# TobiaMarcucci/warm-start-hybrid-mpc

Measured on NVIDIA B200. Metric: bnb_qp_relaxations_per_s, higher is better.
Workload: dtype f64

## Files before the change

warm-start-hybrid-mpc_b200/csrc/qp_device.cuh:

```cuda
#pragma once
#include <cuda_runtime.h>
#include <math.h>
#include <stdint.h>

#ifndef WS_TU
#define WS_TU_HAS(id) 1
#else
#define WS_TU_HAS(id) (WS_TU == (id))
#endif

#ifndef WS_NT
#define WS_NT 256
#endif
#ifndef WS_MAXL
#define WS_MAXL 2
#endif
#define WS_NW (WS_NT / 32)
#ifndef WS_RPT
#define WS_RPT ((384 + WS_NT - 1) / WS_NT)
#endif
#ifndef WS_RRT
#define WS_RRT (256 / WS_NT)
#endif
#ifndef WS_NOINLINE
#define WS_NOINLINE __forceinline__
#endif
#if defined(WS_TU) && WS_TU % 2 == 1
#define WS_WIDE_REGS 1
#else
#define WS_WIDE_REGS 0
#endif
#ifndef WS_CH
#if WS_WIDE_REGS
#define WS_CH 4
#else
#define WS_CH 2
#endif
#endif
#if !WS_WIDE_REGS && !defined(WS_PRICE8)
#define WS_PRICE4 1
#endif
#define WS_OPTIMAL 2
#define WS_INFEASIBLE 3
#define WS_ITER_LIMIT 9
#define WS_REORTH 1e-2
#define WS_LAM_MAX 1e13

#define WS_TID ((int)(threadIdx.x & (WS_NT - 1)))
#define WS_LANE ((int)(threadIdx.x / WS_NT))
#define WS_SYNC() asm volatile("bar.sync %0, %1;" :: "r"(WS_LANE + 1), "n"(WS_NT) : "memory")

struct SmemOff {
    int z, c1, c2, t, u, ls, lam, cw, yc, wv, v, bu, blb, xi, part, red;
    int vf0, vf;
    int pool, pool_sz;
    int irow, iside, ired, iscr;
    int idep;
    int ints;
    int binW, bign, bnadd;
    int bytes;
    int lane_doubles;
    int t_inr, t_vsc, t_sF, t_sG, t_sF1, t_sG1, t_rinfo;
    int tab_doubles;
    int total_bytes;
};

struct DevProblem {
    int nx, nu, nub, nuc, T, nh, nh1, nq, nqT, nr, n, m, mc, nb, ns;
    const double *A, *B, *F, *G, *h, *F1, *G1, *h1, *Q, *R, *QT, *Mmu, *MmuT, *Mrho;
    const double *Mh, *WfT, *nrm, *inr, *vscale, *Eh, *hh, *Rinv, *RinvT, *Kx, *ZmapT, *Linv, *LinvT, *Msq;
    const int *bin_idx;
    int n_elim;
    int search_rule;
    const int *border;
    double eps, tol_p, tol_d, tol_sing, tol_ray, prox_tol;
    int max_iter, max_prox;
    int lanes;
    int ld;
    int np;
    int ns2;
    int gp;
    int hot_cap;
    SmemOff so;
    int n_primal, n_dual, off_lam, off_mu, off_nulb, off_nuub, off_rho, off_sigma;
    int n_rec;
    int node_rule;
};

#ifdef WS_PROF
__device__ unsigned long long g_prof[256];
__device__ __forceinline__ void prof_mark(int id) {
    __shared__ long long s_prof_last;
    if (threadIdx.x == 0) {
        const long long t = clock64();
        atomicAdd(&g_prof[2 * id], (unsigned long long)(t - s_prof_last)); atomicAdd(&g_prof[2 * id + 1], 1ull);
        s_prof_last = clock64();
    }
}
__device__ __forceinline__ void prof_add(int id, int value) {
    if (threadIdx.x == 0) { atomicAdd(&g_prof[2 * id], (unsigned long long)value); atomicAdd(&g_prof[2 * id + 1], 1ull); }
}
#else
#define prof_mark(id) ((void)0)
#define prof_add(id, value) ((void)0)
#endif

__host__ __device__ __forceinline__ int tri_off(int j) { return j * (j + 1) / 2; }

struct SlotPtrs {
    double *Q;
    double *Ri;
    double *lam;
    double *yc;
    int *row;
    int *side;
    int *nW;
};

__host__ __device__ __forceinline__ size_t slot_doubles(int n, int ld) { return (((size_t)n * ld + (size_t)tri_off(n) + (n + 1) + n + 4) + 1) & ~(size_t)1; }
__host__ __device__ __forceinline__ size_t slot_ints(int n) { return 2 * (size_t)(n + 1) + 4; }

__device__ __forceinline__ SlotPtrs slot_ptrs(double *dbase, int *ibase, int slot, int n, int ld) {
    SlotPtrs s;
    double *d = dbase + (size_t)slot * slot_doubles(n, ld);
    int *i = ibase + (size_t)slot * slot_ints(n);
    s.Q = d; d += (size_t)n * ld;
    s.Ri = d; d += tri_off(n);
    s.lam = d; d += n + 1;
    s.yc = d;
    s.row = i; i += n + 1;
    s.side = i; i += n + 1;
    s.nW = i;
    return s;
}

struct Ctx {
    double *smd;
    double *tab;
    double *gQ, *gRi;
    int pg, prp;
};

#define SMV(name) (cx.smd + P.so.name)
#define SMI(name) (reinterpret_cast<int *>(cx.smd + P.so.ints) + P.so.name)
#define SMB(name) (reinterpret_cast<unsigned char *>(cx.smd + P.so.bytes) + P.so.name)
#define TBV(name) (cx.tab + P.so.t_##name)
#define TBI(name) (reinterpret_cast<const int *>(cx.tab + P.so.t_##name))

__device__ __forceinline__ Ctx make_ctx(const DevProblem &P, unsigned char *smem_raw, const SlotPtrs &sp) {
    Ctx cx;
    cx.tab = reinterpret_cast<double *>(smem_raw);
    cx.smd = cx.tab + P.so.tab_doubles + (size_t)WS_LANE * P.so.lane_doubles;
    cx.gQ = sp.Q; cx.gRi = sp.Ri;
    const int hs = P.ns2 >> 1;
    cx.pg = WS_TID / hs; cx.prp = WS_TID - cx.pg * hs;
    return cx;
}

struct Geom {
    int d;
    int d0;
    int he;
    int ldc;
    int ks;
    int triR;
    int G, W;
};

__device__ __forceinline__ Geom load_geom(const DevProblem &P, const Ctx &cx) {
    const int *g = SMI(idep);
    Geom q;
    q.d = g[0]; q.d0 = g[2]; q.he = g[3]; q.ldc = g[4]; q.ks = g[5]; q.triR = g[6]; q.G = g[7]; q.W = g[8];
    return q;
}

__device__ __forceinline__ void store_geom(const DevProblem &P, const Ctx &cx, int d) {
    int *g = SMI(idep);
    d = d < P.n_elim ? d : P.n_elim;
    const int d0 = d & ~1, he = (P.np - d0) >> 1, ldc = 2 * (he | 1);
    int ks = P.n - d;
    while (ks > 0 && (size_t)ks * ldc + ((tri_off(ks) + 1) & ~1) > (size_t)P.so.pool_sz) --ks;
    const int G = he <= WS_NT ? (WS_NT / he < 8 ? WS_NT / he : 8) : 1;
    g[0] = d; g[2] = d0; g[3] = he; g[4] = ldc; g[5] = ks; g[6] = (tri_off(ks) + 1) & ~1; g[7] = G; g[8] = WS_NT / G;
}

__device__ __forceinline__ double warp_sum(double x) {
#pragma unroll
    for (int o = 16; o > 0; o >>= 1) x += __shfl_xor_sync(0xffffffffu, x, o);
    return x;
}

#define WS_FULL 0xffffffffu
static_assert(WS_NW == 16 || WS_NW == 8 || WS_NW == 4 || WS_NW == 2, "the two-level reductions assume 2, 4, 8 or 16 warps per CTA");

__device__ __forceinline__ double block_sum(double x, double *red) {
    const int lane = WS_TID & 31, w = WS_TID >> 5;
    x = warp_sum(x);
    WS_SYNC();
    if (lane == 0) red[w] = x;
    WS_SYNC();
    double s = lane < WS_NW ? red[lane] : 0.;
#pragma unroll
    for (int o = WS_NW / 2; o > 0; o >>= 1) s += __shfl_xor_sync(WS_FULL, s, o);
    return __shfl_sync(WS_FULL, s, 0);
}

__device__ __forceinline__ void block_sum2(double &x, double &y, double *red) {
    const int lane = WS_TID & 31, w = WS_TID >> 5;
    x = warp_sum(x); y = warp_sum(y);
    WS_SYNC();
    if (lane == 0) { red[w] = x; red[16 + w] = y; }
    WS_SYNC();
    double s = (lane & 15) < WS_NW ? red[lane] : 0.;
#pragma unroll
    for (int o = 8; o > 0; o >>= 1) s += __shfl_xor_sync(WS_FULL, s, o);
    x = __shfl_sync(WS_FULL, s, 0); y = __shfl_sync(WS_FULL, s, 16);
}

__device__ __forceinline__ bool better_max(double ov, int oi, double val, int idx) {
    return oi >= 0 && (idx < 0 || ov > val || (ov == val && oi < idx));
}

__device__ __forceinline__ void block_argmax(double &val, int &idx, double *red, int *ired) {
    const int lane = WS_TID & 31, w = WS_TID >> 5;
#pragma unroll
    for (int o = 16; o > 0; o >>= 1) {
        const double ov = __shfl_xor_sync(WS_FULL, val, o);
        const int oi = __shfl_xor_sync(WS_FULL, idx, o);
        if (better_max(ov, oi, val, idx)) { val = ov; idx = oi; }
    }
    WS_SYNC();
    if (lane == 0) { red[w] = val; ired[w] = idx; }
    WS_SYNC();
    val = lane < WS_NW ? red[lane] : 0.; idx = lane < WS_NW ? ired[lane] : -1;
#pragma unroll
    for (int o = WS_NW / 2; o > 0; o >>= 1) {
        const double ov = __shfl_xor_sync(WS_FULL, val, o);
        const int oi = __shfl_xor_sync(WS_FULL, idx, o);
        if (better_max(ov, oi, val, idx)) { val = ov; idx = oi; }
    }
    val = __shfl_sync(WS_FULL, val, 0); idx = __shfl_sync(WS_FULL, idx, 0);
}

__device__ __forceinline__ double block_max(double x, double *red) {
    const int lane = WS_TID & 31, w = WS_TID >> 5;
#pragma unroll
    for (int o = 16; o > 0; o >>= 1) x = fmax(x, __shfl_xor_sync(WS_FULL, x, o));
    WS_SYNC();
    if (lane == 0) red[w] = x;
    WS_SYNC();
    double s = lane < WS_NW ? red[lane] : 0.;
#pragma unroll
    for (int o = WS_NW / 2; o > 0; o >>= 1) s = fmax(s, __shfl_xor_sync(WS_FULL, s, o));
    return __shfl_sync(WS_FULL, s, 0);
}

__device__ __forceinline__ void block_argmin(double &val, int &idx, double *red, int *ired) {
    double nv = -val;
    block_argmax(nv, idx, red, ired);
    val = -nv;
}

__device__ __forceinline__ void warp_argmin_sum(double &val, int &idx, double &sum) {
    double nv = -val;
#pragma unroll
    for (int o = 16; o > 0; o >>= 1) {
        const double ov = __shfl_xor_sync(WS_FULL, nv, o);
        const int oi = __shfl_xor_sync(WS_FULL, idx, o);
        sum += __shfl_xor_sync(WS_FULL, sum, o);
        if (better_max(ov, oi, nv, idx)) { nv = ov; idx = oi; }
    }
    val = -nv;
}

__device__ __forceinline__ void block_argmin_sum(double &val, int &idx, double &sum, double *red, int *ired) {
    const int lane = WS_TID & 31, w = WS_TID >> 5;
    double nv = -val;
#pragma unroll
    for (int o = 16; o > 0; o >>= 1) {
        const double ov = __shfl_xor_sync(WS_FULL, nv, o);
        const int oi = __shfl_xor_sync(WS_FULL, idx, o);
        sum += __shfl_xor_sync(WS_FULL, sum, o);
        if (better_max(ov, oi, nv, idx)) { nv = ov; idx = oi; }
    }
    WS_SYNC();
    if (lane == 0) { red[w] = nv; ired[w] = idx; red[16 + w] = sum; }
    WS_SYNC();
    nv = lane < WS_NW ? red[lane] : 0.; idx = lane < WS_NW ? ired[lane] : -1;
    sum = lane < WS_NW ? red[16 + lane] : 0.;
#pragma unroll
    for (int o = WS_NW / 2; o > 0; o >>= 1) {
        const double ov = __shfl_xor_sync(WS_FULL, nv, o);
        const int oi = __shfl_xor_sync(WS_FULL, idx, o);
        sum += __shfl_xor_sync(WS_FULL, sum, o);
        if (better_max(ov, oi, nv, idx)) { nv = ov; idx = oi; }
    }
    val = -__shfl_sync(WS_FULL, nv, 0); idx = __shfl_sync(WS_FULL, idx, 0); sum = __shfl_sync(WS_FULL, sum, 0);
}

template <class Out>
__device__ __forceinline__ void grouped_matvec(const double *__restrict__ M, int ld, int rows, int j0, int j1,
                                      const double *x, double *part, Out out) {
    if (rows <= WS_NT) {
        const int G = WS_NT / rows;
        const int g = WS_TID / rows, i = WS_TID - g * rows;
        if (g < G) {
            double s0 = 0., s1 = 0., s2 = 0., s3 = 0.;
            int j = j0 + g;
            for (; j + 7 * G < j1; j += 8 * G) {
                double w[8];
#pragma unroll
                for (int q = 0; q < 8; ++q) w[q] = __ldg(M + (size_t)(j + q * G) * ld + i);
                s0 += w[0] * x[j] + w[4] * x[j + 4 * G];
                s1 += w[1] * x[j + G] + w[5] * x[j + 5 * G];
                s2 += w[2] * x[j + 2 * G] + w[6] * x[j + 6 * G];
                s3 += w[3] * x[j + 3 * G] + w[7] * x[j + 7 * G];
            }
            for (; j + 3 * G < j1; j += 4 * G) {
                s0 += M[(size_t)j * ld + i] * x[j];
                s1 += M[(size_t)(j + G) * ld + i] * x[j + G];
                s2 += M[(size_t)(j + 2 * G) * ld + i] * x[j + 2 * G];
                s3 += M[(size_t)(j + 3 * G) * ld + i] * x[j + 3 * G];
            }
            for (; j < j1; j += G) s0 += M[(size_t)j * ld + i] * x[j];
            part[g * rows + i] = (s0 + s1) + (s2 + s3);
        }
        WS_SYNC();
        if (WS_TID < rows) {
            double s = part[WS_TID];
            for (int q = 1; q < G; ++q) s += part[q * rows + WS_TID];
            out(WS_TID, s);
        }
        WS_SYNC();
    } else {
        for (int i = WS_TID; i < rows; i += WS_NT) {
            double s0 = 0., s1 = 0., s2 = 0., s3 = 0.;
            int j = j0;
            for (; j + 7 < j1; j += 8) {
                double w[8];
#pragma unroll
                for (int q = 0; q < 8; ++q) w[q] = __ldg(M + (size_t)(j + q) * ld + i);
                s0 += w[0] * x[j] + w[4] * x[j + 4];
                s1 += w[1] * x[j + 1] + w[5] * x[j + 5];
                s2 += w[2] * x[j + 2] + w[6] * x[j + 6];
                s3 += w[3] * x[j + 3] + w[7] * x[j + 7];
            }
            for (; j < j1; ++j) s0 += M[(size_t)j * ld + i] * x[j];
            out(i, (s0 + s1) + (s2 + s3));
        }
        WS_SYNC();
    }
}

__device__ __forceinline__ double *pool_Ri(const DevProblem &P, const Ctx &cx) { return SMV(pool); }
template <bool SM>
__device__ __forceinline__ double *qcol_w(const DevProblem &P, const Ctx &cx, const Geom &g, int j) {
    if (SM) return SMV(pool) + g.triR + j * g.ldc - g.d0;
    return (j < g.ks ? SMV(pool) + g.triR + j * g.ldc : cx.gQ + (size_t)j * P.ld) - g.d0;
}
template <bool SM>
__device__ __forceinline__ double *ricol_w(const DevProblem &P, const Ctx &cx, const Geom &g, int j) {
    if (SM) return SMV(pool) + tri_off(j);
    return (j < g.ks ? SMV(pool) : cx.gRi) + tri_off(j);
}

__device__ __forceinline__ int team_log2(int k) { return k >= WS_NT ? 0 : min(5, 31 - __clz(WS_NT / max(k, 1))); }

__device__ __forceinline__ double team_sum(double s, int lg) {
    for (int o = 32 >> lg; o < 32; o <<= 1) s += __shfl_xor_sync(0xffffffffu, s, o);
    return s;
}

template <bool SM>
__device__ __forceinline__ void qt_dots_t(const DevProblem &P, const Ctx &cx, int k, const double *x, double *out) {
    const Geom gm = load_geom(P, cx);
    const int lg = team_log2(k), ng = 1 << lg, C = 32 >> lg, jw = WS_NT >> lg;
    const int lane = WS_TID & 31, g = lane >> (5 - lg), jl = (WS_TID >> 5) * C + (lane & (C - 1));
    const int p0 = (gm.d0 >> 1) + g, p1 = P.np >> 1;
    const double2 *x2 = reinterpret_cast<const double2 *>(x);
    const int kr = (k + jw - 1) / jw * jw;
    for (int j = jl; j < kr; j += jw) {
        double s0 = 0., s1 = 0.;
        if (j < k) {
            const double2 *q2 = reinterpret_cast<const double2 *>(qcol_w<SM>(P, cx, gm, j));
            for (int p = p0; p < p1; p += ng) { const double2 a = q2[p], b = x2[p]; s0 += a.x * b.x; s1 += a.y * b.y; }
        }
        const double s = team_sum(s0 + s1, lg);
        if (g == 0 && j < k) out[j] = s;
    }
    WS_SYNC();
}

template <bool SM>
__device__ __forceinline__ double q_apply_t(const DevProblem &P, const Ctx &cx, int k, const double *c, const double *zin, double *zout,
                                 double extra = 0., double *extra_sum = nullptr) {
    const Geom gm = load_geom(P, cx);
    double2 *part2 = reinterpret_cast<double2 *>(SMV(part));
    const int G = gm.G, W = gm.W, he = gm.he, dh = gm.d0 >> 1;
    const int grp = WS_TID / W, t = WS_TID - grp * W;
    if (grp < G) {
        for (int pp = t; pp < he; pp += W) {
            double ax = 0., ay = 0., bx = 0., by = 0.;
            int j = grp;
            for (; j + G < k; j += 2 * G) {
                const double2 a = reinterpret_cast<const double2 *>(qcol_w<SM>(P, cx, gm, j))[dh + pp];
                const double2 b = reinterpret_cast<const double2 *>(qcol_w<SM>(P, cx, gm, j + G))[dh + pp];
                const double ca = c[j], cb = c[j + G];
                ax += a.x * ca; ay += a.y * ca; bx += b.x * cb; by += b.y * cb;
            }
            if (j < k) { const double2 a = reinterpret_cast<const double2 *>(qcol_w<SM>(P, cx, gm, j))[dh + pp]; const double ca = c[j]; ax += a.x * ca; ay += a.y * ca; }
            part2[grp * he + pp] = make_double2(ax + bx, ay + by);
        }
    }
    WS_SYNC();
    const double *part = SMV(part);
    double zz = 0.;
    for (int i = WS_TID; i < 2 * he; i += WS_NT) {
        double s = part[i];
        for (int q = 1; q < G; ++q) s += part[q * 2 * he + i];
        const double zi = (zin ? zin[gm.d0 + i] : 0.) - s;
        zout[gm.d0 + i] = zi; zz += zi * zi;
    }
    {
        const int lane = WS_TID & 31, w = WS_TID >> 5;
        double *red = SMV(red) + 72;
        zz = warp_sum(zz); extra = warp_sum(extra);
        if (lane == 0) { red[w] = zz; red[16 + w] = extra; }
        WS_SYNC();
        double sv = (lane & 15) < WS_NW ? red[lane] : 0.;
#pragma unroll
        for (int o = 8; o > 0; o >>= 1) sv += __shfl_xor_sync(WS_FULL, sv, o);
        zz = __shfl_sync(WS_FULL, sv, 0);
        if (extra_sum) *extra_sum = __shfl_sync(WS_FULL, sv, 16);
    }
    return zz;
}

template <bool SM, class Out>
__device__ __forceinline__ void ri_matvec_ep(const DevProblem &P, const Ctx &cx, int k, const double *c, Out out) {
    const Geom gm = load_geom(P, cx);
    const int lg = team_log2(k), ng = 1 << lg, C = 32 >> lg, jw = WS_NT >> lg;
    const int lane = WS_TID & 31, g = lane >> (5 - lg), il = (WS_TID >> 5) * C + (lane & (C - 1));
    const int kr = (k + jw - 1) / jw * jw;
    for (int i = il; i < kr; i += jw) {
        double s0 = 0., s1 = 0.;
        if (i < k) {
            int j = i + g;
            for (; j + ng < k; j += 2 * ng) { s0 += ricol_w<SM>(P, cx, gm, j)[i] * c[j]; s1 += ricol_w<SM>(P, cx, gm, j + ng)[i] * c[j + ng]; }
            if (j < k) s0 += ricol_w<SM>(P, cx, gm, j)[i] * c[j];
        }
        const double sv = team_sum(s0 + s1, lg);
        if (g == 0 && i < k) out(i, sv);
    }
}

template <bool SM>
__device__ __forceinline__ void ri_matvec(const DevProblem &P, const Ctx &cx, int k, const double *c, double *t) {
    ri_matvec_ep<SM>(P, cx, k, c, [&](int i, double s) { t[i] = s; });
    WS_SYNC();
}

template <bool SM>
__device__ __forceinline__ void rit_matvec_t(const DevProblem &P, const Ctx &cx, int k, const double *d, double *u) {
    const Geom gm = load_geom(P, cx);
    const int lg = team_log2(k), ng = 1 << lg, C = 32 >> lg, jw = WS_NT >> lg;
    const int lane = WS_TID & 31, g = lane >> (5 - lg), jl = (WS_TID >> 5) * C + (lane & (C - 1));
    const int kr = (k + jw - 1) / jw * jw;
    for (int j = jl; j < kr; j += jw) {
        double s = 0.;
        if (j < k) { const double *col = ricol_w<SM>(P, cx, gm, j); for (int i = g; i <= j; i += ng) s += col[i] * d[i]; }
        s = team_sum(s, lg);
        if (g == 0 && j < k) u[j] = s;
    }
    WS_SYNC();
}

__device__ __forceinline__ double neg_bound(const DevProblem &P, const Ctx &cx, int r, int s) {
    return -(s > 0 ? SMV(bu)[r] : -SMV(blb)[r - P.mc]);
}

__device__ __forceinline__ void refresh_uv(const DevProblem &P, const Ctx &cx, int k) {
    const Geom gm = load_geom(P, cx);
    const int *row = SMI(irow), *side = SMI(iside);
    for (int i = WS_TID; i < k; i += WS_NT) SMV(cw)[i] = neg_bound(P, cx, row[i], side[i]);
    for (int i = WS_TID; i < P.np; i += WS_NT) SMV(v)[i] = 0.;
    WS_SYNC();
    if (k <= gm.ks) { rit_matvec_t<true>(P, cx, k, SMV(cw), SMV(u)); ri_matvec<true>(P, cx, k, SMV(u), SMV(ls)); q_apply_t<true>(P, cx, k, SMV(u), nullptr, SMV(v)); }
    else { rit_matvec_t<false>(P, cx, k, SMV(cw), SMV(u)); ri_matvec<false>(P, cx, k, SMV(u), SMV(ls)); q_apply_t<false>(P, cx, k, SMV(u), nullptr, SMV(v)); }
}

struct RowEnt { double e[WS_RPT]; };

__device__ __forceinline__ RowEnt load_row_entries(const DevProblem &P, int r, int d, int d0) {
    RowEnt x;
#pragma unroll
    for (int q = 0; q < WS_RPT; ++q) {
        const int i = d0 + WS_TID + q * WS_NT;
        x.e[q] = (i < P.n && i >= d) ? __ldg(P.Mh + (size_t)r * P.n + i) : 0.;
    }
    return x;
}

template <bool SM>
__device__ __forceinline__ int thin_append_t(const DevProblem &P, const Ctx &cx, int &k, int r, int sgn, bool track, const RowEnt *pre = nullptr) {
    const Geom gm = load_geom(P, cx);
    const int n = P.n, d = gm.d;
    if (k >= WS_RRT * WS_NT) return -1;
    double *z = SMV(z), *c1 = SMV(c1), *t = SMV(t);
    const int pb = track ? 30 : 40;
    (void)pb;
    {
        const RowEnt e = pre ? *pre : load_row_entries(P, r, d, gm.d0);
#pragma unroll
        for (int q = 0; q < WS_RPT; ++q) { const int i = gm.d0 + WS_TID + q * WS_NT; if (i < P.np) z[i] = (double)sgn * e.e[q]; }
    }
    WS_SYNC();
    prof_mark(pb);
    qt_dots_t<SM>(P, cx, k, z, c1);
    prof_mark(pb + 1);
    double cu = 0.;
    if (track) for (int j = WS_TID; j < k; j += WS_NT) cu += c1[j] * SMV(u)[j];
    double rho2 = q_apply_t<SM>(P, cx, k, c1, z, z, cu, &cu);
    prof_mark(pb + 2);
    if (k > 0 && rho2 < WS_REORTH * __ldg(P.Msq + (size_t)r * (P.nb + 1) + d)) {
        double *c2 = SMV(c2);
        qt_dots_t<SM>(P, cx, k, z, c2);
        double cu2 = 0.;
        for (int j = WS_TID; j < k; j += WS_NT) { const double dc = c2[j]; c1[j] += dc; if (track) cu2 += dc * SMV(u)[j]; }
        rho2 = q_apply_t<SM>(P, cx, k, c2, z, z, cu2, &cu2);
        cu += cu2;
        prof_mark(pb + 4);
    }
    const bool dep = k >= n - d || rho2 <= P.tol_sing * P.tol_sing;
    const double ir = dep ? 0. : 1. / sqrt(rho2);
    double *qk = qcol_w<SM>(P, cx, gm, k), *rk = ricol_w<SM>(P, cx, gm, k);
    double uk = 0., lk = 0.;
    if (track && !dep) { uk = (neg_bound(P, cx, r, sgn) - cu) * ir; lk = uk * ir; }
    ri_matvec_ep<SM>(P, cx, k, c1, [&](int i, double ti) {
        t[i] = ti;
        if (!dep) { rk[i] = -ti * ir; if (track) SMV(ls)[i] -= ti * lk; }
    });
    if (dep) { WS_SYNC(); prof_mark(pb + 5); return 0; }
    for (int i = gm.d0 + WS_TID; i < P.np; i += WS_NT) {
        const double q = z[i] * ir;
        qk[i] = q;
        if (track) SMV(v)[i] -= q * uk;
    }
    if (WS_TID == 0) {
        rk[k] = ir;
        SMI(irow)[k] = r; SMI(iside)[k] = sgn; SMV(lam)[k] = 0.;
        if (track) { SMV(u)[k] = uk; SMV(ls)[k] = lk; }
    }
    k += 1;
    if (track) WS_SYNC();
    prof_mark(pb + 6);
    return 1;
}

template <bool SM>
__device__ __forceinline__ int thin_remove_t(const DevProblem &P, const Ctx &cx, int &k, int kp) {
    const Geom gm = load_geom(P, cx);
    auto QC = [&](int j) -> double * { return qcol_w<SM>(P, cx, gm, j); };
    auto RC = [&](int j) -> double * { return ricol_w<SM>(P, cx, gm, j); };
    const int lane = WS_TID & 31, w = WS_TID >> 5, tid = WS_TID;
    double *gc = SMV(c2), *gs = SMV(cw), *u = SMV(u);
    int *row = SMI(irow), *side = SMI(iside), *flag = SMI(ired) + 32;
    if (tid == 0) *flag = 0x7fffffff;
    prof_add(100, k - 1 - kp);
    prof_add(101, k);
    if (kp == k - 1) {
        const double ul = u[kp];
        const double *qk = QC(kp);
        for (int i = gm.d0 + tid; i < P.np; i += WS_NT) SMV(v)[i] += qk[i] * ul;
        const double *rl = RC(kp);
        for (int i = tid; i < kp; i += WS_NT) SMV(ls)[i] -= rl[i] * ul;
        k -= 1;
        WS_SYNC();
        prof_mark(50);
        return -1;
    }
    if (w == 0) {
        const double wkp = RC(kp)[kp];
        double run = 0.;
        for (int b = kp; b < k; b += 32) {
            const int j = b + lane;
            const double wj = j < k ? RC(j)[kp] : 0.;
            double s = wj * wj;
#pragma unroll
            for (int o = 1; o < 32; o <<= 1) { const double y = __shfl_up_sync(0xffffffffu, s, o); if (lane >= o) s += y; }
            s += run;
            double excl = __shfl_up_sync(0xffffffffu, s, 1);
            if (lane == 0) excl = run;
            if (j > kp && j < k) {
                const double isj = 1. / sqrt(s);
                const double tau = (j - 1 == kp) ? wkp : sqrt(excl);
                gc[j - 1] = wj * isj; gs[j - 1] = -tau * isj;
            }
            run = __shfl_sync(0xffffffffu, s, 31);
        }
    }
    int rw[WS_RRT], sd[WS_RRT]; double lm[WS_RRT];
#pragma unroll
    for (int q = 0; q < WS_RRT; ++q) {
        const int ts = kp + 1 + tid + q * WS_NT;
        rw[q] = 0; sd[q] = 0; lm[q] = 0.;
        if (ts < k) { rw[q] = row[ts]; sd[q] = side[ts]; lm[q] = SMV(lam)[ts]; }
    }
    int qr[WS_RPT]; double qcarry[WS_RPT];
#pragma unroll
    for (int q = 0; q < WS_RPT; ++q) { const int i = gm.d0 + tid + q * WS_NT; qr[q] = i < P.np ? i : -1; }
    int rr[WS_RRT], ro[WS_RRT]; double rcarry[WS_RRT], ls_old[WS_RRT];
#pragma unroll
    for (int q = 0; q < WS_RRT; ++q) {
        const int r = WS_NT - 1 - tid + q * WS_NT;
        rr[q] = r < k - 1 ? r : -1;
        ro[q] = r < kp ? r : r + 1;
    }
    const int nq1 = (2 * gm.he + 31) & ~31;
    const bool uth = tid == (nq1 < WS_NT ? nq1 : 0);
    const double big = 1. / P.tol_sing;
    WS_SYNC();
    prof_mark(51);
#pragma unroll
    for (int q = 0; q < WS_RRT; ++q) {
        const int ts = kp + 1 + tid + q * WS_NT;
        if (ts < k) { row[ts - 1] = rw[q]; side[ts - 1] = sd[q]; SMV(lam)[ts - 1] = lm[q]; }
    }
#pragma unroll
    for (int q = 0; q < WS_RPT; ++q) qcarry[q] = qr[q] >= 0 ? QC(kp)[qr[q]] : 0.;
#pragma unroll
    for (int q = 0; q < WS_RRT; ++q) {
        rcarry[q] = (rr[q] >= 0 && ro[q] <= kp) ? RC(kp)[ro[q]] : 0.;
    }
    double ucarry = uth ? u[kp] : 0.;
    for (int i0 = kp; i0 < k - 1; i0 += WS_CH) {
        double b[WS_RRT][WS_CH];
#pragma unroll
        for (int q = 0; q < WS_RRT; ++q) if (rr[q] >= 0) {
#pragma unroll
            for (int c = 0; c < WS_CH; ++c) { const int i = i0 + c; b[q][c] = (i < k - 1 && ro[q] <= i + 1) ? RC(i + 1)[ro[q]] : 0.; }
        }
        WS_SYNC();
        prof_mark(54);
#pragma unroll
        for (int q = 0; q < WS_RRT; ++q) if (rr[q] >= 0 && ro[q] <= i0 + WS_CH) {
#pragma unroll
            for (int c = 0; c < WS_CH; ++c) {
                const int i = i0 + c;
                if (i < k - 1) {
                    const double cs = gc[i], sn = gs[i];
                    const double o = cs * rcarry[q] + sn * b[q][c];
                    rcarry[q] = -sn * rcarry[q] + cs * b[q][c];
                    if (rr[q] <= i) {
                        RC(i)[rr[q]] = o;
                        if (rr[q] == i && fabs(o) >= big) atomicMin(flag, rr[q]);
                    }
                }
            }
        }
        const int iend = (i0 + WS_CH < k - 1) ? i0 + WS_CH : k - 1;
        prof_mark(55);
#pragma unroll
        for (int q = 0; q < WS_RPT; ++q) if (qr[q] >= 0) {
            for (int i = i0; i < iend; ++i) {
                const double bq = QC(i + 1)[qr[q]];
                const double cs = gc[i], sn = gs[i];
                QC(i)[qr[q]] = cs * qcarry[q] + sn * bq;
                qcarry[q] = -sn * qcarry[q] + cs * bq;
            }
        }
        if (uth) {
            for (int i = i0; i < iend; ++i) {
                const double bu_ = u[i + 1];
                const double cs = gc[i], sn = gs[i];
                u[i] = cs * ucarry + sn * bu_;
                ucarry = -sn * ucarry + cs * bu_;
            }
        }
        prof_mark(56);
    }
    if (uth) SMV(red)[40] = ucarry;
#pragma unroll
    for (int q = 0; q < WS_RRT; ++q) ls_old[q] = rr[q] >= 0 ? SMV(ls)[ro[q]] : 0.;
    k -= 1;
    WS_SYNC();
    prof_mark(52);
#pragma unroll
    for (int q = 0; q < WS_RPT; ++q) if (qr[q] >= 0) SMV(v)[qr[q]] += qcarry[q] * SMV(red)[40];
#pragma unroll
    for (int q = 0; q < WS_RRT; ++q) if (rr[q] >= 0) SMV(ls)[rr[q]] = ls_old[q] - rcarry[q] * SMV(red)[40];
    const int bad = *flag;
    WS_SYNC();
    prof_mark(53);
    return bad == 0x7fffffff ? -1 : bad;
}

__device__ __forceinline__ int thin_append(const DevProblem &P, const Ctx &cx, int &k, int r, int sgn, bool track, const RowEnt *pre = nullptr) {
    const Geom gm = load_geom(P, cx);
    return k < gm.ks ? thin_append_t<true>(P, cx, k, r, sgn, track, pre) : thin_append_t<false>(P, cx, k, r, sgn, track, pre);
}
__device__ __forceinline__ int thin_remove(const DevProblem &P, const Ctx &cx, int &k, int kp) {
    const Geom gm = load_geom(P, cx);
    return k <= gm.ks ? thin_remove_t<true>(P, cx, k, kp) : thin_remove_t<false>(P, cx, k, kp);
}

__device__ __forceinline__ void ws_remove(const DevProblem &P, const Ctx &cx, int &k, int kp) {
    signed char *inW = reinterpret_cast<signed char *>(SMB(binW));
    int pos = kp;
    do {
        if (WS_TID == 0) inW[SMI(irow)[pos]] = 0;
        WS_SYNC();
        pos = thin_remove(P, cx, k, pos);
    } while (pos >= 0);
}

template <class Skip, class Fn>
__device__ __forceinline__ void price_rows(const DevProblem &P, const Ctx &cx, const double *x, int c0, int pid, Skip skip, Fn f) {
    const int n = P.n, m = P.m, mc = P.mc, nx = P.nx, nu = P.nu;
    const int hs = P.ns2 >> 1;
    double *xi = SMV(xi);
    {
        double2 *part2 = reinterpret_cast<double2 *>(SMV(part));
        if (cx.pg < P.gp) {
            const double2 *w2 = reinterpret_cast<const double2 *>(P.WfT) + cx.prp;
            double ax = 0., ay = 0., bx = 0., by = 0., ex = 0., ey = 0., dx = 0., dy = 0.;
            int c = c0 + cx.pg;
            const int G = P.gp;
#ifndef WS_PRICE4
            for (; c + 7 * G < n; c += 8 * G) {
                double2 w[8];
#pragma unroll
                for (int q = 0; q < 8; ++q) w[q] = __ldg(w2 + (size_t)(c + q * G) * hs);
#pragma unroll
                for (int q = 0; q < 8; q += 4) {
                    const double xa = x[c + q * G], xb = x[c + (q + 1) * G], xe = x[c + (q + 2) * G], xd = x[c + (q + 3) * G];
                    ax += w[q].x * xa; ay += w[q].y * xa; bx += w[q + 1].x * xb; by += w[q + 1].y * xb;
                    ex += w[q + 2].x * xe; ey += w[q + 2].y * xe; dx += w[q + 3].x * xd; dy += w[q + 3].y * xd;
                }
            }
#endif
            for (; c + 3 * G < n; c += 4 * G) {
                const double2 a = __ldg(w2 + (size_t)c * hs), b = __ldg(w2 + (size_t)(c + G) * hs),
                              e = __ldg(w2 + (size_t)(c + 2 * G) * hs), d = __ldg(w2 + (size_t)(c + 3 * G) * hs);
                const double xa = x[c], xb = x[c + G], xe = x[c + 2 * G], xd = x[c + 3 * G];
                ax += a.x * xa; ay += a.y * xa; bx += b.x * xb; by += b.y * xb;
                ex += e.x * xe; ey += e.y * xe; dx += d.x * xd; dy += d.y * xd;
            }
            for (; c < n; c += G) { const double2 a = __ldg(w2 + (size_t)c * hs); const double xa = x[c]; ax += a.x * xa; ay += a.y * xa; }
            part2[cx.pg * hs + cx.prp] = make_double2((ax + bx) + (ex + dx), (ay + by) + (ey + dy));
        }
        if (P.gp == 0) {
            double2 *xi2 = reinterpret_cast<double2 *>(xi);
            for (int pp = WS_TID; pp < hs; pp += WS_NT) {
                const double2 *w2 = reinterpret_cast<const double2 *>(P.WfT) + pp;
                double ax = 0., ay = 0., bx = 0., by = 0.;
                int c = c0;
                for (; c + 1 < n; c += 2) {
                    const double2 a = __ldg(w2 + (size_t)c * hs), b = __ldg(w2 + (size_t)(c + 1) * hs);
                    const double xa = x[c], xb = x[c + 1];
                    ax += a.x * xa; ay += a.y * xa; bx += b.x * xb; by += b.y * xb;
                }
                if (c < n) { const double2 a = __ldg(w2 + (size_t)c * hs); const double xa = x[c]; ax += a.x * xa; ay += a.y * xa; }
                xi2[pp] = make_double2(ax + bx, ay + by);
            }
        }
        WS_SYNC();
        if (P.gp > 0) {
            const double *part = SMV(part);
            for (int r = WS_TID; r < P.ns2; r += WS_NT) {
                double s = part[r];
                for (int q = 1; q < P.gp; ++q) s += part[q * P.ns2 + r];
                xi[r] = s;
            }
        }
        WS_SYNC();
        prof_mark(pid);
    }
    const int *rinfo = TBI(rinfo);
    const double *inr = TBV(inr);
    for (int r = WS_TID; r < m; r += WS_NT) {
        if (skip(r)) continue;
        double s;
        const int info = rinfo[r];
        if (r < mc) {
            const int t = info >> 16, i = info & 0xffff;
            const bool last = t == P.T - 1;
            const int rs = last ? P.nh1 : P.nh;
            const double *Fr = (last ? TBV(sF1) : TBV(sF)) + i;
            const double *Gr = (last ? TBV(sG1) : TBV(sG)) + i;
            const double *zt = xi + t * nu;
            double s0 = 0., s1 = 0.;
            int c = 0;
            for (; c + 1 < nu; c += 2) { s0 += Gr[c * rs] * zt[c]; s1 += Gr[(c + 1) * rs] * zt[c + 1]; }
            if (c < nu) s0 += Gr[c * rs] * zt[c];
            if (t > 0) {
                const double *xt = xi + n + (t - 1) * nx;
                c = 0;
                for (; c + 1 < nx; c += 2) { s0 += Fr[c * rs] * xt[c]; s1 += Fr[(c + 1) * rs] * xt[c + 1]; }
                if (c < nx) s0 += Fr[c * rs] * xt[c];
            }
            s = s0 + s1;
        } else {
            s = xi[info];
        }
        f(r, s * inr[r]);
    }
}


__device__ __forceinline__ uint32_t smem_u32(const void *p) { return (uint32_t)__cvta_generic_to_shared(p); }
__device__ __forceinline__ void mbar_init(uint64_t *bar, int count) {
    asm volatile("mbarrier.init.shared::cta.b64 [%0], %1;" :: "r"(smem_u32(bar)), "r"(count) : "memory");
}
__device__ __forceinline__ void mbar_expect_tx(uint64_t *bar, uint32_t bytes) {
    asm volatile("mbarrier.arrive.expect_tx.shared::cta.b64 _, [%0], %1;" :: "r"(smem_u32(bar)), "r"(bytes) : "memory");
}
__device__ __forceinline__ void mbar_wait(uint64_t *bar, uint32_t parity) {
    uint32_t done;
    do {
        asm volatile("{ .reg .pred p; mbarrier.try_wait.parity.shared::cta.b64 p, [%1], %2; selp.u32 %0, 1, 0, p; }"
                     : "=r"(done) : "r"(smem_u32(bar)), "r"(parity) : "memory");
    } while (!done);
}
__device__ __forceinline__ void fence_async_smem() { asm volatile("fence.proxy.async.shared::cta;" ::: "memory"); }
__device__ __forceinline__ void bulk_g2s(void *sdst, const void *gsrc, uint32_t bytes, uint64_t *bar) {
    asm volatile("cp.async.bulk.shared::cluster.global.mbarrier::complete_tx::bytes [%0], [%1], %2, [%3];"
                 :: "r"(smem_u32(sdst)), "l"(gsrc), "r"(bytes), "r"(smem_u32(bar)) : "memory");
}
__device__ __forceinline__ void bulk_s2g(void *gdst, const void *ssrc, uint32_t bytes) {
    asm volatile("cp.async.bulk.global.shared::cta.bulk_group [%0], [%1], %2;" :: "l"(gdst), "r"(smem_u32(ssrc)), "r"(bytes) : "memory");
}
__device__ __forceinline__ void bulk_commit_wait() {
    asm volatile("cp.async.bulk.commit_group;" ::: "memory");
    asm volatile("cp.async.bulk.wait_group 0;" ::: "memory");
}
#define WS_MBAR (reinterpret_cast<uint64_t *>(SMV(red) + 100))

__device__ __forceinline__ void init_shared_tables(const DevProblem &P, const Ctx &cx) {
    const int nt = blockDim.x, t0 = threadIdx.x;
    double *sF = cx.tab + P.so.t_sF, *sG = cx.tab + P.so.t_sG, *sF1 = cx.tab + P.so.t_sF1, *sG1 = cx.tab + P.so.t_sG1;
    for (int e = t0; e < P.nh * P.nx; e += nt) { const int i = e / P.nx, c = e - i * P.nx; sF[c * P.nh + i] = P.F[e]; }
    for (int e = t0; e < P.nh * P.nu; e += nt) { const int i = e / P.nu, c = e - i * P.nu; sG[c * P.nh + i] = P.G[e]; }
    for (int e = t0; e < P.nh1 * P.nx; e += nt) { const int i = e / P.nx, c = e - i * P.nx; sF1[c * P.nh1 + i] = P.F1[e]; }
    for (int e = t0; e < P.nh1 * P.nu; e += nt) { const int i = e / P.nu, c = e - i * P.nu; sG1[c * P.nh1 + i] = P.G1[e]; }
    int *rinfo = reinterpret_cast<int *>(cx.tab + P.so.t_rinfo);
    for (int r = t0; r < P.m; r += nt) {
        (cx.tab + P.so.t_inr)[r] = P.inr[r]; (cx.tab + P.so.t_vsc)[r] = P.vscale[r];
        int info;
        if (r < P.mc) { int t = r / P.nh; if (t > P.T - 1) t = P.T - 1; info = (t << 16) | (r - t * P.nh); }
        else info = P.bin_idx[r - P.mc];
        rinfo[r] = info;
    }
    for (int i = WS_TID; i < P.np + 2; i += WS_NT) { SMV(z)[i] = 0.; SMV(v)[i] = 0.; SMV(wv)[i] = 0.; SMV(yc)[i] = 0.; }
    for (int i = WS_TID; i < P.ns2; i += WS_NT) SMV(xi)[i] = 0.;
    if (WS_TID == 0) { store_geom(P, cx, 0); SMI(idep)[9] = 0; mbar_init(WS_MBAR, 1); fence_async_smem(); }
    __syncthreads();
}

__device__ __forceinline__ void load_slot(const DevProblem &P, const Ctx &cx, const SlotPtrs &sp, int &k, bool reset) {
    const int n = P.n;
    if (reset) {
        for (int i = WS_TID; i < n; i += WS_NT) SMV(yc)[i] = 0.;
        k = 0;
    } else {
        k = *sp.nW;
        for (int i = WS_TID; i < n; i += WS_NT) SMV(yc)[i] = sp.yc[i];
        for (int i = WS_TID; i < k; i += WS_NT) { SMI(irow)[i] = sp.row[i]; SMI(iside)[i] = sp.side[i]; SMV(lam)[i] = sp.lam[i]; }
    }
    WS_SYNC();
}

__device__ __forceinline__ void store_slot(const DevProblem &P, const Ctx &cx, const SlotPtrs &sp, int k) {
    const int n = P.n;
    for (int i = WS_TID; i < n; i += WS_NT) sp.yc[i] = SMV(yc)[i];
    for (int i = WS_TID; i < k; i += WS_NT) { sp.row[i] = SMI(irow)[i]; sp.side[i] = SMI(iside)[i]; sp.lam[i] = SMV(lam)[i]; }
    if (WS_TID == 0) *sp.nW = k;
    WS_SYNC();
}

template <class Y>
__device__ __forceinline__ void load_ws_from_multipliers(const DevProblem &P, const Ctx &cx, Y ysigned, const double *yc0, int &k) {
    const int lane = WS_TID & 31, w = WS_TID >> 5;
    int *wsum = SMI(ired);
    int *row = SMI(irow), *side = SMI(iside);
    double *lam = SMV(lam);
    const int d = SMI(idep)[0];
    for (int i = WS_TID; i < P.n; i += WS_NT) SMV(yc)[i] = yc0 ? yc0[i] : 0.;
    int base = 0;
    for (int r0 = 0; r0 < P.m; r0 += WS_NT) {
        const int r = r0 + WS_TID;
        double yv = 0.;
        if (r < P.m) yv = ysigned(r);
        const int keep = yv != 0. && base < P.n && !(r >= P.mc && r - P.mc < d);
        const unsigned bal = __ballot_sync(0xffffffffu, keep);
        WS_SYNC();
        if (lane == 0) wsum[w] = __popc(bal);
        WS_SYNC();
        int pre = base, tot = 0;
        for (int q = 0; q < WS_NW; ++q) { const int c = wsum[q]; if (q < w) pre += c; tot += c; }
        const int idx = pre + __popc(bal & ((1u << lane) - 1u));
        if (keep && idx < P.n) { row[idx] = r; side[idx] = yv > 0. ? 1 : -1; lam[idx] = fabs(yv) * P.nrm[r]; }
        base += tot;
    }
    k = base < P.n ? base : P.n;
    WS_SYNC();
#ifndef WS_NO_SORT
    {
        int *scr = SMI(iscr); double *tmp = SMV(cw);
        for (int i = WS_TID; i < k; i += WS_NT) {
            const double li = lam[i];
            int rank = 0;
            for (int j = 0; j < k; ++j) { const double lj = lam[j]; rank += (lj > li || (lj == li && j < i)) ? 1 : 0; }
            scr[i] = rank | (row[i] << 10) | (side[i] > 0 ? (1 << 30) : 0);
            tmp[i] = li;
        }
        WS_SYNC();
        for (int i = WS_TID; i < k; i += WS_NT) {
            const int e = scr[i], rank = e & 0x3ff;
            row[rank] = (e >> 10) & 0xfffff; side[rank] = (e >> 30) & 1 ? 1 : -1; lam[rank] = tmp[i];
        }
        WS_SYNC();
    }
#endif
}

__device__ __forceinline__ void rebuild_factor(const DevProblem &P, const Ctx &cx, int &k) {
    const Geom gm = load_geom(P, cx);
    signed char *inW = reinterpret_cast<signed char *>(SMB(binW));
    unsigned char *ign = SMB(bign), *nadd = SMB(bnadd);
    const int d = gm.d;
    for (int r = WS_TID; r < P.m; r += WS_NT) { inW[r] = 0; ign[r] = (r >= P.mc && r - P.mc < d) ? 3 : 0; nadd[r] = 0; }
    const int k0 = k;
    double *lam0 = SMV(cw), *lam = SMV(lam);
    int *row = SMI(irow), *side = SMI(iside);
    int *row0 = SMI(iscr);
    WS_SYNC();
    for (int i = WS_TID; i < k0; i += WS_NT) { row0[i] = row[i] * 2 + (side[i] > 0 ? 1 : 0); lam0[i] = lam[i]; }
    WS_SYNC();
    k = 0;
    RowEnt pre = load_row_entries(P, k0 > 0 ? row0[0] >> 1 : 0, d, gm.d0);
    for (int i = 0; i < k0; ++i) {
        const int r = row0[i] >> 1, s = (row0[i] & 1) ? 1 : -1;
        const RowEnt cur = pre;
        if (i + 1 < k0) pre = load_row_entries(P, row0[i + 1] >> 1, d, gm.d0);
        if (r >= P.mc && r - P.mc < d) continue;
        if (thin_append(P, cx, k, r, s, false, &cur) > 0) {
            if (WS_TID == 0) { lam[k - 1] = lam0[i]; inW[r] = (signed char)s; }
        }
    }
    WS_SYNC();
}

__device__ __forceinline__ void save_factor(const DevProblem &P, const Ctx &cx, const SlotPtrs &sp, int k) {
    const Geom gm = load_geom(P, cx);
#ifdef WS_NO_TMA
    for (int e = WS_TID; e < tri_off(k); e += WS_NT) sp.Ri[e] = SMV(pool)[e];
    for (int e = WS_TID; e < k * gm.ldc; e += WS_NT) sp.Q[e] = (SMV(pool) + gm.triR)[e];
    if (WS_TID == 0) *sp.nW = k;
#else
    if (WS_TID == 0) {
        fence_async_smem();
        bulk_s2g(sp.Ri, SMV(pool), (uint32_t)(((tri_off(k) + 1) & ~1) * 8));
        bulk_s2g(sp.Q, SMV(pool) + gm.triR, (uint32_t)(k * gm.ldc * 8));
        bulk_commit_wait();
        *sp.nW = k;
    }
#endif
    for (int i = WS_TID; i < k; i += WS_NT) { sp.row[i] = SMI(irow)[i]; sp.side[i] = SMI(iside)[i]; sp.lam[i] = SMV(lam)[i]; }
    WS_SYNC();
}

__device__ __forceinline__ void restore_factor(const DevProblem &P, const Ctx &cx, const SlotPtrs &sp, int &k) {
    const Geom gm = load_geom(P, cx);
    signed char *inW = reinterpret_cast<signed char *>(SMB(binW));
    unsigned char *ign = SMB(bign), *nadd = SMB(bnadd);
    const int d = gm.d;
    k = *sp.nW;
    int *phase = SMI(idep) + 9;
    const uint32_t par = (uint32_t)*phase;
    WS_SYNC();
#ifdef WS_NO_TMA
    for (int e = WS_TID; e < tri_off(k); e += WS_NT) SMV(pool)[e] = sp.Ri[e];
    for (int e = WS_TID; e < k * gm.ldc; e += WS_NT) (SMV(pool) + gm.triR)[e] = sp.Q[e];
#else
    if (WS_TID == 0) {
        const uint32_t bR = (uint32_t)(((tri_off(k) + 1) & ~1) * 8), bQ = (uint32_t)(k * gm.ldc * 8);
        fence_async_smem();
        mbar_expect_tx(WS_MBAR, bR + bQ);
        bulk_g2s(SMV(pool), sp.Ri, bR, WS_MBAR);
        bulk_g2s(SMV(pool) + gm.triR, sp.Q, bQ, WS_MBAR);
        *phase = (int)(par ^ 1u);
    }
#endif
    for (int r = WS_TID; r < P.m; r += WS_NT) { inW[r] = 0; ign[r] = (r >= P.mc && r - P.mc < d) ? 3 : 0; nadd[r] = 0; }
    for (int i = WS_TID; i < k; i += WS_NT) { SMI(irow)[i] = sp.row[i]; SMI(iside)[i] = sp.side[i]; SMV(lam)[i] = sp.lam[i]; }
    WS_SYNC();
    for (int i = WS_TID; i < k; i += WS_NT) inW[SMI(irow)[i]] = (signed char)SMI(iside)[i];
#ifndef WS_NO_TMA
    mbar_wait(WS_MBAR, par);
#endif
    WS_SYNC();
}


__device__ __forceinline__ void set_node_prefix(const DevProblem &P, const Ctx &cx, const double *lb, const double *ub) {
    double far = 0.;
// ... 293 lines not shown
```

Baseline: 467,700.

## Sweep Givens rotations per thread without chunk barriers and compact R afterwards

For non-wide-register builds, the thin QR removal now has each thread run its Givens sweep over Q rows, R entries and u in one loop. This drops the per-chunk block barriers used by the chunked sweep. Because each thread now owns its R entries in place, a new ri_compact pass shifts the packed triangular R columns after the sweep, mapping elements to columns with a float rsqrt-based tri_col. Rotations are also written as explicit fma/mul forms in both paths. The cost is an extra pass over R plus one barrier per compaction chunk, and the float column estimate relies on its off-by-one correction.

```diff
diff --git a/warm-start-hybrid-mpc_b200/csrc/qp_device.cuh b/warm-start-hybrid-mpc_b200/csrc/qp_device.cuh
--- a/warm-start-hybrid-mpc_b200/csrc/qp_device.cuh
+++ b/warm-start-hybrid-mpc_b200/csrc/qp_device.cuh
@@ -37,6 +37,10 @@
 #define WS_CH 2
 #endif
 #endif
+#ifndef WS_SWEEP_INPLACE
+#define WS_SWEEP_INPLACE (!WS_WIDE_REGS)
+#endif
+#define WS_CPT 4
 #if !WS_WIDE_REGS && !defined(WS_PRICE8)
 #define WS_PRICE4 1
 #endif
@@ -106,6 +110,12 @@
 #endif
 
 __host__ __device__ __forceinline__ int tri_off(int j) { return j * (j + 1) / 2; }
+__device__ __forceinline__ int tri_col(int e) {
+    const float y = 8.f * (float)e + 1.f;
+    int j = (int)((y * rsqrtf(y) - 1.f) * .5f);
+    if (tri_off(j + 1) <= e) ++j; else if (tri_off(j) > e) --j;
+    return j;
+}
 
 struct SlotPtrs {
     double *Q;
@@ -558,7 +568,7 @@
 }
 
 template <bool SM>
-__device__ __forceinline__ int thin_remove_t(const DevProblem &P, const Ctx &cx, int &k, int kp) {
+__device__ __forceinline__ bool thin_remove_t(const DevProblem &P, const Ctx &cx, int &k, int kp) {
     const Geom gm = load_geom(P, cx);
     auto QC = [&](int j) -> double * { return qcol_w<SM>(P, cx, gm, j); };
     auto RC = [&](int j) -> double * { return ricol_w<SM>(P, cx, gm, j); };
@@ -577,7 +587,7 @@
         k -= 1;
         WS_SYNC();
         prof_mark(50);
-        return -1;
+        return false;
     }
     if (w == 0) {
         const double wkp = RC(kp)[kp];
@@ -626,6 +636,60 @@
         const int ts = kp + 1 + tid + q * WS_NT;
         if (ts < k) { row[ts - 1] = rw[q]; side[ts - 1] = sd[q]; SMV(lam)[ts - 1] = lm[q]; }
     }
+#if WS_SWEEP_INPLACE
+#pragma unroll
+    for (int q = 0; q < WS_RPT; ++q) {
+        double qa = 0.;
+        if (qr[q] >= 0) {
+            double *qc = QC(kp) + qr[q];
+            qa = *qc;
+            #pragma unroll 1
+            for (int i = kp; i < k - 1; ++i) {
+                double *qn = SM ? qc + gm.ldc : QC(i + 1) + qr[q];
+                const double bq = *qn;
+                const double cs = gc[i], sn = gs[i];
+                *qc = __fma_rn(sn, bq, __dmul_rn(cs, qa));
+                qa = __fma_rn(cs, bq, -__dmul_rn(sn, qa));
+                qc = qn;
+            }
+        }
+        qcarry[q] = qa;
+    }
+#pragma unroll
+    for (int q = 0; q < WS_RRT; ++q) {
+        double rc = 0.;
+        if (rr[q] >= 0) {
+            const int x = ro[q] - kp;
+            int i = kp + WS_CH * ((max(x, 1) - 1) / WS_CH);
+            if (x < 0) rc = RC(kp)[ro[q]];
+            double *p = RC(i + 1) + ro[q];
+            #pragma unroll 1
+            for (; i < k - 1; ++i) {
+                const double b = ro[q] <= i + 1 ? *p : 0.;
+                const double cs = gc[i], sn = gs[i];
+                const double o = __fma_rn(cs, rc, __dmul_rn(sn, b));
+                rc = __fma_rn(cs, b, -__dmul_rn(sn, rc));
+                if (rr[q] <= i) {
+                    *p = o;
+                    if (rr[q] == i && fabs(o) >= big) atomicMin(flag, rr[q]);
+                }
+                p = SM ? p + (i + 2) : RC(i + 2) + ro[q];
+            }
+        }
+        rcarry[q] = rc;
+    }
+    if (uth) {
+        double ucarry = u[kp];
+        #pragma unroll 1
+        for (int i = kp; i < k - 1; ++i) {
+            const double bu_ = u[i + 1];
+            const double cs = gc[i], sn = gs[i];
+            u[i] = __fma_rn(cs, ucarry, __dmul_rn(sn, bu_));
+            ucarry = __fma_rn(cs, bu_, -__dmul_rn(sn, ucarry));
+        }
+        SMV(red)[40] = ucarry;
+    }
+#else
 #pragma unroll
     for (int q = 0; q < WS_RPT; ++q) qcarry[q] = qr[q] >= 0 ? QC(kp)[qr[q]] : 0.;
 #pragma unroll
@@ -649,8 +713,8 @@
                 const int i = i0 + c;
                 if (i < k - 1) {
                     const double cs = gc[i], sn = gs[i];
-                    const double o = cs * rcarry[q] + sn * b[q][c];
-                    rcarry[q] = -sn * rcarry[q] + cs * b[q][c];
+                    const double o = __fma_rn(cs, rcarry[q], __dmul_rn(sn, b[q][c]));
+                    rcarry[q] = __fma_rn(cs, b[q][c], -__dmul_rn(sn, rcarry[q]));
                     if (rr[q] <= i) {
                         RC(i)[rr[q]] = o;
                         if (rr[q] == i && fabs(o) >= big) atomicMin(flag, rr[q]);
@@ -665,21 +729,22 @@
             for (int i = i0; i < iend; ++i) {
                 const double bq = QC(i + 1)[qr[q]];
                 const double cs = gc[i], sn = gs[i];
-                QC(i)[qr[q]] = cs * qcarry[q] + sn * bq;
-                qcarry[q] = -sn * qcarry[q] + cs * bq;
+                QC(i)[qr[q]] = __fma_rn(sn, bq, __dmul_rn(cs, qcarry[q]));
+                qcarry[q] = __fma_rn(cs, bq, -__dmul_rn(sn, qcarry[q]));
             }
         }
         if (uth) {
             for (int i = i0; i < iend; ++i) {
                 const double bu_ = u[i + 1];
                 const double cs = gc[i], sn = gs[i];
-                u[i] = cs * ucarry + sn * bu_;
-                ucarry = -sn * ucarry + cs * bu_;
+                u[i] = __fma_rn(cs, ucarry, __dmul_rn(sn, bu_));
+                ucarry = __fma_rn(cs, bu_, -__dmul_rn(sn, ucarry));
             }
         }
         prof_mark(56);
     }
     if (uth) SMV(red)[40] = ucarry;
+#endif
 #pragma unroll
     for (int q = 0; q < WS_RRT; ++q) ls_old[q] = rr[q] >= 0 ? SMV(ls)[ro[q]] : 0.;
     k -= 1;
@@ -689,10 +754,28 @@
     for (int q = 0; q < WS_RPT; ++q) if (qr[q] >= 0) SMV(v)[qr[q]] += qcarry[q] * SMV(red)[40];
 #pragma unroll
     for (int q = 0; q < WS_RRT; ++q) if (rr[q] >= 0) SMV(ls)[rr[q]] = ls_old[q] - rcarry[q] * SMV(red)[40];
-    const int bad = *flag;
-    WS_SYNC();
-    prof_mark(53);
-    return bad == 0x7fffffff ? -1 : bad;
+    return true;
+}
+
+__device__ __forceinline__ void ri_compact(const DevProblem &P, const Ctx &cx, int k, int kp) {
+    const Geom gm = load_geom(P, cx);
+    const int e1 = tri_off(k);
+    for (int e0 = tri_off(kp); e0 < e1; e0 += WS_CPT * WS_NT) {
+        double cv[WS_CPT], *dst[WS_CPT];
+#pragma unroll
+        for (int q = 0; q < WS_CPT; ++q) {
+            const int e = e0 + WS_TID + q * WS_NT;
+            dst[q] = nullptr; cv[q] = 0.;
+            if (e < e1) {
+                const int i = tri_col(e), r = e - tri_off(i);
+                dst[q] = ricol_w<false>(P, cx, gm, i) + r;
+                cv[q] = ricol_w<false>(P, cx, gm, i + 1)[r + (r >= kp)];
+            }
+        }
+        WS_SYNC();
+#pragma unroll
+        for (int q = 0; q < WS_CPT; ++q) if (dst[q]) *dst[q] = cv[q];
+    }
 }
 
 __device__ __forceinline__ int thin_append(const DevProblem &P, const Ctx &cx, int &k, int r, int sgn, bool track, const RowEnt *pre = nullptr) {
@@ -701,7 +784,14 @@
 }
 __device__ __forceinline__ int thin_remove(const DevProblem &P, const Ctx &cx, int &k, int kp) {
     const Geom gm = load_geom(P, cx);
-    return k <= gm.ks ? thin_remove_t<true>(P, cx, k, kp) : thin_remove_t<false>(P, cx, k, kp);
+    if (!(k <= gm.ks ? thin_remove_t<true>(P, cx, k, kp) : thin_remove_t<false>(P, cx, k, kp))) return -1;
+#if WS_SWEEP_INPLACE
+    ri_compact(P, cx, k, kp);
+#endif
+    const int bad = SMI(ired)[32];
+    WS_SYNC();
+    prof_mark(53);
+    return bad == 0x7fffffff ? -1 : bad;
 }
 
 __device__ __forceinline__ void ws_remove(const DevProblem &P, const Ctx &cx, int &k, int kp) {
```

Measured after the change: 478,000, median of 6. 2.2% higher.
